# feldroop/genedex

Measured on AMD Instinct MI355X. Metric: queries/sec (count+locate), hg38-scale text, 100M len-50 reads, higher is better.
Workload: dtype u32

## Files before the change

genedex_amd/csrc/search.hip:

```cpp
#include <atomic>
#include <cstdlib>
#include <string>
#include <type_traits>

#include "common.hpp"
#include "kernels.hpp"

namespace gdx {

namespace {

constexpr int kBlock = 256;

struct QueryWindow {
    const uint64_t *words;
    uint64_t cur;
    uint64_t next;
    uint64_t cur_word;
    uint64_t first_word;

    __device__ __forceinline__ void init(const uint8_t *qbuf, uint64_t begin, uint64_t pos)
    {
        words = reinterpret_cast<const uint64_t *>(qbuf);
        first_word = begin >> 3;
// ... 1744 lines not shown
                        a0 = w.l0;
                        a1 = w.l1;
                        a2 = w.l2;
                    }
                    const uint32_t n_lv = rem >> 3 < static_cast<uint32_t>(kLevels) ? rem >> 3 : static_cast<uint32_t>(kLevels);
                    const uint32_t qa = a0, qb = a1 & 0xffffu, qc = __builtin_amdgcn_alignbit(a2, a1, 16);
                    const uint32_t qok = vl & ((1u << n_lv) - 1u);
                    const uint32_t row = lo + sub < hi ? lo + sub : hi - 1u;
                    const u32x4 *tab = static_cast<const u32x4 *>(ix.jump);
                    const u32x4 *pa = kJump == 8 ? tab + (row >> 1) : tab + static_cast<uint64_t>(row) * (kJump / 16);
                    u32x4 e0, e1;
                    load_round2<0>(pa, pa + 1, kHalf2 ? __ballot(true) : 0ull, e0, e1);
                    uint32_t valid, da, db = 0, dc = 0;
                    if (kJump == 8) {
                        const uint32_t ew = (row & 1u) ? e0.w : e0.y;
                        da = (ew ^ qa) & 0xffffu;
                        valid = ew >> 16;
                    } else {
                        da = e0.z ^ qa;
                        db = (e0.w ^ qb) & 0xffffu;
                        valid = e0.w >> 16;
                        if (kHalf2) dc = e1.w ^ qc;
                    }
                    uint32_t good = (da & 0xffffu) == 0u ? 1u : 0u;
                    if (kLevels >= 2) good |= (da >> 16) == 0u ? 2u : 0u;
                    if (kHalf2) {
                        good |= db == 0u ? 4u : 0u;
                        good |= (dc & 0xffffu) == 0u ? 8u : 0u;
                    }
                    good &= valid & qok;
                    const uint32_t lvl = static_cast<uint32_t>(__builtin_ctz(~good | (1u << kLevels)));
                    const uint32_t best = group_max<kGroup>(lvl);
                    if (best == 0u) {
                        jump_ok = false;
                        continue;
                    }
                    const bool mine = lvl == best;
                    uint32_t target = kJump == 8 ? ((row & 1u) ? e0.z : e0.x) : e0.x;
                    if (kLevels >= 2) target = best == 2u ? e0.y : target;
                    if (kHalf2) {
                        target = best == 3u ? e1.x : target;
                        target = best == 4u ? e1.y : target;
                    }
                    lo = group_min<kGroup>(mine ? target : 0xffffffffu);
                    hi = group_max<kGroup>(mine ? target : 0u) + 1u;
                    rem -= best * kJumpSymbols;
                    shift += best;
                    continue;
                }
                const uint32_t e = sel4(shift >> 1, w.l0, w.l1, w.l2, w.l3);
                const uint32_t f = sel4((shift >> 1) + 1u, w.l0, w.l1, w.l2, w.l3);
                const uint32_t lv2 = (shift & 1u) ? ((e & 0xffff0000u) | (f & 0xffffu)) : __builtin_amdgcn_alignbit(e, e, 16);
                const uint32_t x = lv2 << (2u * part);
                const bool two = rem >= 2u;
                {
                    const uint32_t t_last = part + (two ? 1u : 0u);
                    const uint32_t need = (part < w.s0 ? 1u : 2u) | (t_last < w.s0 ? 1u : 2u);
                    if ((v8 & need) != need) {
                        bail = true;
                        break;
                    }
                }
                const uint32_t c1 = (x >> 30) + 1u, c2 = two ? ((x >> 28) & 3u) + 1u : 0u;
                const uint32_t line_lo = lo >> kPairLineShift, line_hi = hi >> kPairLineShift;
                const bool second = line_hi != line_lo;
                const u32x4 *pa = ix.pair_lines + (static_cast<uint64_t>(line_lo) << 3) + sub;
                const u32x4 *pb = ix.pair_lines + (static_cast<uint64_t>(line_hi) << 3) + sub;
                u32x4 a[2], b[2];
                load_round4<0>(pa, pa + kGroup, pb, pb + kGroup, __ballot(true), __ballot(second), a[0], a[1], b[0], b[1]);
                if (!second) {
                    b[0] = a[0];
                    b[1] = a[1];
                }
                bool stepped = false;
                if (two) {
                    const uint32_t pair = (c2 - 1u) * 4u + (c1 - 1u);
                    const uint32_t bits_x = (c1 & 1u) | ((c1 & 2u) << 7) | ((c1 & 4u) << 14) | ((c2 & 1u) << 24);
                    const uint32_t bits_y = ((c2 >> 1) & 1u) | ((c2 & 4u) << 6);
                    const uint32_t nx = ~(bits_x * 0xffu);
                    const uint32_t ny = ~(bits_y * 0xffu) & 0xffffu;
                    uint32_t plo = 0, phi = 0;
#pragma unroll
                    for (int k = 0; k < 2; k++) {
                        plo += PairTable::pair_partial(a[k], sub + k * kGroup, pair, nx, ny, lo);
                        phi += PairTable::pair_partial(b[k], sub + k * kGroup, pair, nx, ny, hi);
                    }
                    const uint32_t nlo = quad_sum(plo), nhi = quad_sum(phi);
                    if (nlo != nhi) {
                        lo = nlo;
                        hi = nhi;
                        rem -= 2u;
                        part += 2u;
                        stepped = true;
                    }
                }
                if (!stepped) {
                    const uint32_t bits_x = (c1 & 1u) | ((c1 & 2u) << 7) | ((c1 & 4u) << 14);
                    const uint32_t nx = ~(bits_x * 0xffu) & 0xffffffu;
                    uint32_t plo = 0, phi = 0;
#pragma unroll
                    for (int k = 0; k < 2; k++) {
                        plo += PairTable::single_partial(a[k], sub + k * kGroup, c1, nx, lo);
                        phi += PairTable::single_partial(b[k], sub + k * kGroup, c1, nx, hi);
                    }
                    lo = quad_sum(plo);
                    hi = quad_sum(phi);
                    rem -= 1u;
                    part += 1u;
                }
                shift += part >> 3;
                part &= 7u;
            }
            if (writer) {
                if (bail) {
                    s_left[atomicAdd(&s_nleft, 1u)] = q;
                } else {
                    const bool unchanged = kCursor && len == 0u;
                    if (out_start && !unchanged) out_start[q] = lo;
                    if (out_end && !unchanged) out_end[q] = hi;
                    if (out_count) out_count[q] = hi - lo;
                    if (!kCursor && out_status) out_status[q] = 0;
                    if (kCursor && ca.active_out != nullptr && lo != hi && more_left) s_alive[slot] = q;
                }
            }
        }
        }
        __syncthreads();
        const uint32_t n_left = s_nleft;
        if (threadIdx.x == 0 && n_left != 0u) s_left_base = atomicAdd(n_leftover, n_left);
        __syncthreads();
        for (uint32_t i = threadIdx.x; i < n_left; i += kBlock) leftover[s_left_base + i] = s_left[i];
        __syncthreads();
        if (threadIdx.x == 0) s_nleft = 0;
        if (kCursor && ca.active_out != nullptr)
            flush_live_ordered(s_alive, cnt, s_alive_part, &s_alive_base, ca.active_out, ca.n_active_out);
    }
}

struct VerifyView {
    const uint2 *top;
    const u32x4 *text_units;
    const uint32_t *sa_full;
    const void *jump;
    const u32x4 *lines;
    const uint32_t *sb_offsets, *count, *sa_samples, *border_keys, *border_vals;
    const uint8_t *io_to_dense;
    uint32_t top_depth, n, n_texts, sa_inv, sa_rot, sa_limit, max_rows;
    uint32_t perm_code_lo, perm_code_hi, perm_exp_lo, perm_exp_hi, perm_mask;
    const u32x4 *seed;
    uint32_t seed_buckets, seed_k, seed_tag_bits;
    const u32x4 *seed_pairs, *seed_quads;
};

template <int kXlate, bool kSeed>
__global__ __launch_bounds__(kBlock) __attribute__((amdgpu_waves_per_eu(7, 7))) void search_verify_kernel4(
    VerifyView vv, const uint8_t *__restrict__ qbuf, const uint64_t *__restrict__ qbeg, const uint64_t *__restrict__ qend,
    uint64_t nq, uint32_t *__restrict__ out_count, uint8_t *__restrict__ out_status, uint4 *out_rec,
    uint32_t range, uint32_t *__restrict__ leftover, uint32_t *__restrict__ n_leftover,
    const uint32_t *__restrict__ list, const uint32_t *__restrict__ n_list,
    uint32_t ulen,
    const uint4 *state,
    uint32_t wide_to_list,
    uint32_t state_packed)
{
    constexpr int kGroup = 4;
    __shared__ uint8_t s_dense[256];
    __shared__ uint32_t s_count[8];
    __shared__ uint32_t s_left[kMaxRange];
    __shared__ uint32_t s_nleft, s_left_base;
    if (list != nullptr) nq = *n_list;
    if (static_cast<uint64_t>(blockIdx.x) * range >= nq) return;
    if (kXlate == 0)
        for (int i = threadIdx.x; i < 256; i += kBlock) s_dense[i] = vv.io_to_dense[i];
    if (threadIdx.x < 8) s_count[threadIdx.x] = threadIdx.x < 6 ? vv.count[threadIdx.x] : 0u;
    if (threadIdx.x == 0) s_nleft = 0;
    __syncthreads();
    IndexView ix{};
    ix.lines = vv.lines;
    ix.sb_offsets = vv.sb_offsets;
    ix.sa_inv = vv.sa_inv;
    ix.sa_rot = vv.sa_rot;
    ix.sa_limit = vv.sa_limit;
    const bool writer = (threadIdx.x % kGroup) == 0;
    const uint32_t sub = threadIdx.x & (kGroup - 1u);
    const uint32_t depth = vv.top_depth;
    const uint64_t n_ranges = (nq + range - 1) / range;
    for (uint64_t rg = blockIdx.x; rg < n_ranges; rg += gridDim.x) {
        const uint64_t base = rg * range;
        const uint32_t cnt = nq - base < range ? static_cast<uint32_t>(nq - base) : range;
        for (uint32_t slot = threadIdx.x / kGroup; slot < cnt; slot += kBlock / kGroup) {
            const uint32_t q = list != nullptr ? list[base + slot] : static_cast<uint32_t>(base + slot);
            uint4 st = make_uint4(0u, 0u, 0u, 0u);
            if (kSeed && state != nullptr) st = state[q];
            const bool from_state = kSeed && state != nullptr && state_packed != 0u && wide_to_list != 0u && (st.y & kStatePacked) != 0u &&
                                    (st.y & kStateSymbolsMask) <= 32u;
            const uint64_t begin = from_state ? 0ull : query_begin(qbeg, ulen, q);
            const uint64_t len = from_state ? 0ull : query_end(qend, ulen, q) - begin;
            bool bail = from_state ? false
                                   : (kSeed ? !(len >= vv.seed_k && len < (1ull << 21)) : !(len >= 16u && len >= depth && len < (1ull << 21)));
            uint32_t lo = 0, hi = 0, rem = 0;
            const uint64_t *wbase = query_words<kXlate>(qbuf, begin);
            const uint32_t off0 = static_cast<uint32_t>(begin & 7u);
            FastWindow w = {0u, 0u, 0u, 0u, 0u, 8u};
            uint32_t shift = 0, part = 0;
            bool single = false;
            bool single_ok = false;
            uint32_t pos = 0;
            bool resumed = false;
            const uint64_t state_codes = (static_cast<uint64_t>(st.z) << 32) | st.w;
            if (from_state && (st.y & kStatePair) != 0u && (st.y >> kStateRowsShift) > 2u) {
                const u32x4 *qr = vv.seed_quads + 4ull * st.x;
                const u32x4 q0 = qr[0], q1 = qr[1], q2 = qr[2], q3 = qr[3];
                const uint32_t n_v = st.y & kStateSymbolsMask, rows_q = st.y >> kStateRowsShift;
                const uint64_t vm64 = n_v == 32u ? ~0ull : ~0ull << (2u * (32u - n_v));
                const uint32_t p_me = sel4(sub, q0.x, q0.y, q0.z, q0.w);
                const uint64_t t_me = (static_cast<uint64_t>(sel4(sub, q1.y, q1.w, q2.y, q2.w)) << 32) | sel4(sub, q1.x, q1.z, q2.x, q2.z);
                uint32_t alive_q = (sub < rows_q && ((state_codes ^ t_me) & vm64) == 0ull && p_me >= n_v) ? 1u << sub : 0u;
                alive_q |= static_cast<uint32_t>(__builtin_amdgcn_mov_dpp(static_cast<int>(alive_q), 0xB1, 0xF, 0xF, true));
                alive_q |= static_cast<uint32_t>(__builtin_amdgcn_mov_dpp(static_cast<int>(alive_q), 0x4E, 0xF, 0xF, true));
                if (writer) {
                    const uint32_t n_alive = static_cast<uint32_t>(__popc(alive_q));
                    uint4 rec;
                    if (n_alive == 0u) {
                        rec = make_uint4(0u, 0u, 0xffffffffu, 0u);
                    } else if (n_alive <= 2u) {
                        const uint32_t f = static_cast<uint32_t>(__builtin_ctz(alive_q));
                        const uint32_t h1 = sel4(f, q0.x, q0.y, q0.z, q0.w) - n_v;
                        if (n_alive == 1u) {
                            rec = make_uint4(0u, 1u, h1, kRecResolved);
                        } else {
                            const uint32_t g = static_cast<uint32_t>(__builtin_ctz(alive_q & (alive_q - 1u)));
                            const uint32_t h2 = sel4(g, q0.x, q0.y, q0.z, q0.w) - n_v;
                            rec = make_uint4(h2, h2 + 2u, h1, kRecResolved);
                        }
                    } else {
                        rec = make_uint4(q3.x, q3.x + n_alive, alive_q, (n_v & 0x1fffffu) | kRecMasked);
                    }
                    if (out_rec) out_rec[q] = rec;
                    if (out_count) out_count[q] = rec.y - rec.x;
                    if (out_status) out_status[q] = 0;
                }
                continue;
            }
            if (from_state && (st.y & kStatePair) != 0u) {
                const u32x4 *pr = vv.seed_pairs + 2ull * st.x;
                const u32x4 r0 = pr[0], r1 = pr[1];
                const uint32_t n_v = st.y & kStateSymbolsMask;
                const uint64_t vm64 = n_v == 32u ? ~0ull : ~0ull << (2u * (32u - n_v));
                const uint64_t t1 = (static_cast<uint64_t>(r0.w) << 32) | r0.z, t2 = (static_cast<uint64_t>(r1.y) << 32) | r1.x;
                const bool ok1 = ((state_codes ^ t1) & vm64) == 0ull && r0.x >= n_v, ok2 = ((state_codes ^ t2) & vm64) == 0ull && r0.y >= n_v;
                if (writer) {
                    const uint32_t h1 = r0.x - n_v, h2 = r0.y - n_v;
                    uint4 rec;
                    if (ok1 && ok2) rec = make_uint4(h2, h2 + 2u, h1, kRecResolved);
                    else if (ok1 || ok2) rec = make_uint4(0u, 1u, ok1 ? h1 : h2, kRecResolved);
                    else rec = make_uint4(0u, 0u, 0xffffffffu, 0u);
                    if (out_rec) out_rec[q] = rec;
                    if (out_count) out_count[q] = rec.y - rec.x;
                    if (out_status) out_status[q] = 0;
                }
                continue;
            }
            if (from_state) {
                resumed = true;
                lo = st.x;
                hi = lo + (st.y >> kStateRowsShift);
                rem = st.y & kStateSymbolsMask;
            } else if (kSeed && !bail && state != nullptr) {
                const bool plain = state_packed == 0u && st.w == 1u;
                const bool p_rows = state_packed != 0u && (st.y & kStatePacked) != 0u, p_wide = state_packed != 0u && (st.y & kStatePlain) != 0u;
                if (plain || p_rows || p_wide) {
                    resumed = true;
                    rem = static_cast<uint32_t>(len);
                    w = fast_window<kXlate>(vv, s_dense, wbase, off0, rem, sub);
                    lo = st.x;
                    hi = plain ? st.y : (p_rows ? lo + (st.y >> kStateRowsShift) : st.z);
                    rem = plain ? st.z : st.y & kStateSymbolsMask;
                    shift = vv.seed_k >> 3;
                    part = vv.seed_k & 7u;
                }
            }
            if (kSeed && !bail && !resumed) {
                rem = static_cast<uint32_t>(len);
                w = fast_window<kXlate>(vv, s_dense, wbase, off0, rem, sub);
                const uint32_t k = vv.seed_k;
                const uint32_t n_look = rem < k + 32u ? rem : k + 32u;
                const uint32_t n_words = n_look <= w.s0 ? 1u : 1u + ((n_look - w.s0 + 7u) >> 3);
                if ((w.valid8 & ((1u << n_words) - 1u)) != (1u << n_words) - 1u) {
                    bail = true;
                } else {
                    const uint32_t w0 = __builtin_amdgcn_alignbit(w.l0, w.l0, 16), w1 = __builtin_amdgcn_alignbit(w.l1, w.l1, 16);
                    const uint32_t w2 = __builtin_amdgcn_alignbit(w.l2, w.l2, 16), w3 = __builtin_amdgcn_alignbit(w.l3, w.l3, 16);
                    const uint64_t key = ((static_cast<uint64_t>(w0) << 32) | w1) >> (64u - 2u * k);
                    uint32_t tag;
                    uint32_t b = seed_home(key, vv.seed_tag_bits, vv.seed_buckets, tag);
                    uint32_t ex, ey, ez, ew;
                    for (uint32_t d = 0;; d++) {
                        const u32x4 *bp = vv.seed + (static_cast<uint64_t>(b) << 3) + 2u * sub;
                        const u32x4 e0 = bp[0], e1 = bp[1];
                        const uint32_t want = tag | (d << kSeedDispShift);
                        const bool m0 = (e0.x & kSeedMatchMask) == want, m1 = (e1.x & kSeedMatchMask) == want;
                        const u32x4 es = m0 ? e0 : e1;
                        const bool m = m0 || m1;
                        ex = m ? (es.x | kSeedFound) : (e0.x & kSeedOverflow);
                        ey = m ? es.y : 0u;
                        ez = m ? es.z : 0u;
                        ew = m ? es.w : 0u;
                        ex |= static_cast<uint32_t>(__builtin_amdgcn_mov_dpp(static_cast<int>(ex), 0xB1, 0xF, 0xF, true));
                        ey |= static_cast<uint32_t>(__builtin_amdgcn_mov_dpp(static_cast<int>(ey), 0xB1, 0xF, 0xF, true));
                        ez |= static_cast<uint32_t>(__builtin_amdgcn_mov_dpp(static_cast<int>(ez), 0xB1, 0xF, 0xF, true));
                        ew |= static_cast<uint32_t>(__builtin_amdgcn_mov_dpp(static_cast<int>(ew), 0xB1, 0xF, 0xF, true));
                        ex |= static_cast<uint32_t>(__builtin_amdgcn_mov_dpp(static_cast<int>(ex), 0x4E, 0xF, 0xF, true));
                        ey |= static_cast<uint32_t>(__builtin_amdgcn_mov_dpp(static_cast<int>(ey), 0x4E, 0xF, 0xF, true));
                        ez |= static_cast<uint32_t>(__builtin_amdgcn_mov_dpp(static_cast<int>(ez), 0x4E, 0xF, 0xF, true));
                        ew |= static_cast<uint32_t>(__builtin_amdgcn_mov_dpp(static_cast<int>(ew), 0x4E, 0xF, 0xF, true));
                        if ((ex & kSeedFound) != 0u || (ex & kSeedOverflow) == 0u || d >= kSeedMaxDisp) break;
                        b = b + 1u == vv.seed_buckets ? 0u : b + 1u;
                    }
                    rem -= k;
                    shift = k >> 3;
                    part = k & 7u;
                    if ((ex & kSeedFound) == 0u) {
                        lo = hi = 0u;
                    } else if ((ex & kSeedKind) != 0u) {
                        lo = ey;
                        hi = ez;
                    } else {
                        single = true;
                        lo = 0u;
                        hi = 1u;
                        pos = ey;
                        uint32_t qh, ql;
                        const uint32_t sh = 32u - 2u * (k & 15u);
                        if (k == 16u) {
                            qh = w1;
                            ql = w2;
                        } else if (k < 16u) {
                            qh = __builtin_amdgcn_alignbit(w0, w1, sh);
                            ql = __builtin_amdgcn_alignbit(w1, w2, sh);
                        } else {
                            qh = __builtin_amdgcn_alignbit(w1, w2, sh);
                            ql = __builtin_amdgcn_alignbit(w2, w3, sh);
                        }
                        const uint32_t n_v = rem < 32u ? rem : 32u;
                        const uint64_t vm64 = n_v == 32u ? ~0ull : ~(~0ull >> (2u * n_v));
                        const uint64_t qcode = (static_cast<uint64_t>(qh) << 32) | ql;
                        const uint64_t tcode = (static_cast<uint64_t>(ew) << 32) | ez;
                        const uint32_t v_code = (ex >> kSeedPartialShift) & 3u;
                        const uint32_t n_text = (ex & kSeedPartial) == 0u ? 0xffffffffu : (v_code == 0u ? (ez & 63u) : 29u + v_code);
                        single_ok = ((qcode ^ tcode) & vm64) == 0ull && pos >= rem && rem <= n_text;
                    }
                }
            }
            if (!kSeed && !bail) {
                rem = static_cast<uint32_t>(len);
                w = fast_window<kXlate>(vv, s_dense, wbase, off0, rem, sub);
                const uint32_t need = (w.s0 == 8u ? 1u : 3u) | (depth > 8u ? (w.s0 == 8u ? 2u : 6u) : 0u);
                if ((w.valid8 & need) != need) {
                    bail = true;
                } else {
                    const uint2 e = vv.top[__builtin_amdgcn_alignbit(w.l0, w.l0, 16) >> (32u - 2u * depth)];
                    lo = e.x;
                    hi = e.y;
                    rem -= depth;
                    shift = depth >> 3;
                    part = depth & 7u;
                }
            }
            if (wide_to_list != 0u && !bail && rem > 0u && hi - lo > vv.max_rows) bail = true;
            while (!bail && rem > 0u && hi - lo > vv.max_rows) {
                if (shift > 6u) {
                    w = fast_window<kXlate>(vv, s_dense, wbase, off0, rem, sub);
                    shift = 0;
                    part = 0;
                }
                const uint32_t v8 = w.valid8 >> shift;
                if ((v8 & (part < w.s0 ? 1u : 2u)) == 0u) {
                    bail = true;
                    break;
                }
                const uint32_t e = sel4(shift >> 1, w.l0, w.l1, w.l2, w.l3);
                const uint32_t lv = (shift & 1u) ? e >> 16 : e & 0xffffu;
                const uint32_t c = ((lv >> (14u - 2u * part)) & 3u) + 1u;
                uint32_t rlo, rhi;
                QuadLineTable::rank2(ix, c, lo, hi, rlo, rhi);
                lo = s_count[c] + rlo;
                hi = s_count[c] + rhi;
                rem--;
                part++;
                shift += part >> 3;
                part &= 7u;
            }
            const uint32_t rows = hi - lo;
            uint32_t alive = 0;
            uint32_t pair_first = 0, pair_second = 0;
            bool pair = false;
            if (kSeed && single && !bail && (rem <= 32u || !single_ok)) {
                alive = single_ok ? 1u : 0u;
            } else if (!bail && rem > 0u && rows != 0u) {
                const bool real = sub < rows;
                const uint32_t row = real ? lo + sub : lo;
                if (kSeed && single) {
                } else if (vv.sa_full != nullptr) {
                    pos = vv.sa_full[row];
                } else if (vv.jump != nullptr) {
                    pos = static_cast<const uint32_t *>(vv.jump)[static_cast<uint64_t>(row) * 8u + 6u];
                } else {
                    uint32_t r_ = row, steps = 0;
                    for (;;) {
                        uint32_t slot_;
                        if (sampled_slot(ix, r_, slot_)) {
                            pos = vv.sa_samples[slot_] + steps;
                            break;
                        }
                        uint32_t rk;
                        const uint32_t c = LineTable::symbol_and_rank(ix, r_, rk);
                        if (c == 0) {
                            pos = vv.border_vals[lower_bound_u32(vv.border_keys, vv.n_texts, r_)] + steps;
                            break;
                        }
                        r_ = vv.count[c] + rk;
                        steps++;
                    }
                }
                bool ok = real && pos >= rem;
                uint32_t rem_v = rem;
                bool first = part == 0u && shift <= 3u;
                if (kSeed && single) {
                    rem_v = rem - 32u;
                    first = false;
                }
                while (rem_v > 0u) {
                    const uint32_t n_v = rem_v < 32u ? rem_v : 32u;
                    uint64_t qcode;
                    if (from_state) {
                        qcode = state_codes;
                    } else {
                        if (!first) {
                            w = fast_window<kXlate>(vv, s_dense, wbase, off0, rem_v, sub);
                            shift = 0;
                        }
                        first = false;
                        const uint32_t v8 = w.valid8 >> shift;
                        const uint32_t vl = v8 & (w.s0 == 8u ? 0xffu : (v8 >> 1));
                        const uint32_t n_full = n_v >> 3, n_tail = n_v & 7u;
                        bool clean = (vl & ((1u << n_full) - 1u)) == ((1u << n_full) - 1u);
                        if (n_tail != 0u) clean = clean && ((v8 >> n_full) & 1u) != 0u && (n_tail <= w.s0 || ((v8 >> (n_full + 1u)) & 1u) != 0u);
                        if (!clean) {
                            bail = true;
                            break;
                        }
                        uint32_t a0, a1;
                        if (shift == 0u) {
                            a0 = w.l0;
                            a1 = w.l1;
                        } else if (shift == 1u) {
                            a0 = __builtin_amdgcn_alignbit(w.l1, w.l0, 16);
                            a1 = __builtin_amdgcn_alignbit(w.l2, w.l1, 16);
                        } else if (shift == 2u) {
                            a0 = w.l1;
                            a1 = w.l2;
                        } else {
                            a0 = __builtin_amdgcn_alignbit(w.l2, w.l1, 16);
                            a1 = __builtin_amdgcn_alignbit(w.l3, w.l2, 16);
                        }
                        qcode = (static_cast<uint64_t>(__builtin_amdgcn_alignbit(a0, a0, 16)) << 32) |
                                static_cast<uint64_t>(__builtin_amdgcn_alignbit(a1, a1, 16));
                    }
                    const uint64_t s0 = static_cast<uint64_t>(pos) - rem + rem_v + 32u * kTextPadUnits - 32u;
                    const uint32_t b = static_cast<uint32_t>(s0 & 31u);
                    const u32x4 *tu = vv.text_units + (s0 >> 5);
                    const u32x4 u0 = ok ? tu[0] : u32x4{0u, 0u, 0u, 0u};
                    const u32x4 u1 = (ok && b != 0u) ? tu[1] : u32x4{0u, 0u, 0u, 0u};
                    const uint64_t c0 = static_cast<uint64_t>(u0.x) | (static_cast<uint64_t>(u0.y) << 32);
                    const uint64_t c1 = static_cast<uint64_t>(u1.x) | (static_cast<uint64_t>(u1.y) << 32);
                    const uint64_t tcode = b ? (c0 >> (2u * b)) | (c1 << (64u - 2u * b)) : c0;
                    const uint32_t tmask = b ? (u0.z >> b) | (u1.z << (32u - b)) : u0.z;
                    const uint64_t vm64 = n_v == 32u ? ~0ull : ~0ull << (2u * (32u - n_v));
                    const uint32_t vm32 = n_v == 32u ? ~0u : ~0u << (32u - n_v);
                    ok = ok && ((qcode ^ tcode) & vm64) == 0ull && (tmask & vm32) == 0u;
                    rem_v -= n_v;
                }
                alive = (ok && !bail) ? 1u << sub : 0u;
                alive |= static_cast<uint32_t>(__builtin_amdgcn_mov_dpp(static_cast<int>(alive), 0xB1, 0xF, 0xF, true));
                alive |= static_cast<uint32_t>(__builtin_amdgcn_mov_dpp(static_cast<int>(alive), 0x4E, 0xF, 0xF, true));
                const int mine = static_cast<int>(pos - rem);
                const uint32_t o0 = static_cast<uint32_t>(__builtin_amdgcn_mov_dpp(mine, 0x00, 0xF, 0xF, true));
                const uint32_t o1 = static_cast<uint32_t>(__builtin_amdgcn_mov_dpp(mine, 0x55, 0xF, 0xF, true));
                const uint32_t o2 = static_cast<uint32_t>(__builtin_amdgcn_mov_dpp(mine, 0xAA, 0xF, 0xF, true));
                const uint32_t o3 = static_cast<uint32_t>(__builtin_amdgcn_mov_dpp(mine, 0xFF, 0xF, 0xF, true));
                if (__popc(alive) == 2) {
                    const uint32_t f = static_cast<uint32_t>(__builtin_ctz(alive)), g = static_cast<uint32_t>(__builtin_ctz(alive & (alive - 1u)));
                    pair_first = sel4(f, o0, o1, o2, o3);
                    pair_second = sel4(g, o0, o1, o2, o3);
                    pair = true;
                }
            }
            if (writer) {
                if (bail) {
                    s_left[atomicAdd(&s_nleft, 1u)] = q;
                    if (kSeed && state_packed != 0u && resumed && out_rec) out_rec[q] = make_uint4(lo, hi, rem, 1u);
                } else {
                    uint4 rec;
                    if (kSeed && single) {
                        rec = alive ? make_uint4(0u, 1u, pos - rem, kRecResolved) : make_uint4(0u, 0u, 0xffffffffu, 0u);
                    } else if (rem == 0u || rows == 0u) {
                        rec = make_uint4(lo, hi, 0xffffffffu, 0u);
                    } else if (rows == 1u) {
                        rec = alive ? make_uint4(lo, lo + 1u, pos - rem, kRecResolved) : make_uint4(lo, lo, 0xffffffffu, 0u);
                    } else if (pair) {
                        rec = make_uint4(pair_second, pair_second + 2u, pair_first, kRecResolved);
                    } else {
                        rec = make_uint4(lo, lo + static_cast<uint32_t>(__popc(alive)), alive, (rem & 0x1fffffu) | kRecMasked);
                    }
                    if (out_rec) out_rec[q] = rec;
                    if (out_count) out_count[q] = rec.y - rec.x;
                    if (out_status) out_status[q] = 0;
                }
            }
        }
        __syncthreads();
        const uint32_t n_left = s_nleft;
        if (threadIdx.x == 0 && n_left != 0u) s_left_base = atomicAdd(n_leftover, n_left);
        __syncthreads();
        for (uint32_t i = threadIdx.x; i < n_left; i += kBlock) leftover[s_left_base + i] = s_left[i];
        __syncthreads();
        if (threadIdx.x == 0) s_nleft = 0;
    }
}

struct SeedView {
    const u32x4 *seed;
    const u32x4 *text_units;
    const uint32_t *isa;
    const uint8_t *io_to_dense;
    uint32_t buckets, k, tag_bits;
    uint32_t perm_code_lo, perm_code_hi, perm_exp_lo, perm_exp_hi, perm_mask;
    uint32_t n = 0;
};

template <int kXlate, bool kExact, bool kCursor = false>
__global__ __launch_bounds__(kBlock) __attribute__((amdgpu_waves_per_eu(8, 8))) void search_seed_kernel4(
    SeedView sv, const uint8_t *__restrict__ qbuf, const uint64_t *__restrict__ qbeg, const uint64_t *__restrict__ qend,
    uint64_t nq, uint32_t *__restrict__ out_count, uint8_t *__restrict__ out_status, uint4 *__restrict__ out_rec,
    uint32_t *__restrict__ out_start, uint32_t *__restrict__ out_end,
    uint32_t range, uint32_t *__restrict__ leftover, uint32_t *__restrict__ n_leftover,
    uint4 *__restrict__ state,
    uint32_t *__restrict__ out_compact,
    uint32_t *__restrict__ long_list, uint32_t *__restrict__ n_long, uint2 *__restrict__ long_state, uint32_t long_stride,
    uint32_t state_packed,
    uint32_t ulen,
    CursorArgs ca)
{
    static_assert(!kCursor || kExact, "cursor chunks are exact searches");
    constexpr uint32_t kGroup = 4, kGroups = kBlock / kGroup;
    constexpr uint32_t kNoQuery = 0xffffffffu;
    __shared__ uint8_t s_dense[256];
    __shared__ uint16_t s_left[kMaxRange], s_long[kMaxRange];
    __shared__ uint32_t s_nleft, s_left_base, s_nlong, s_long_base;
    __shared__ uint32_t s_alive[kCursor ? kCursorRange : 1];
    __shared__ uint32_t s_alive_part[kCursor ? kBlock : 1];
    __shared__ uint32_t s_alive_base;
    if (kXlate == 0)
        for (int i = threadIdx.x; i < 256; i += kBlock) s_dense[i] = sv.io_to_dense[i];
    if (kCursor)
        for (uint32_t i = threadIdx.x; i < kCursorRange; i += kBlock) s_alive[i] = kDeadCursor;
    if (threadIdx.x == 0) s_nleft = s_nlong = 0;
    __syncthreads();
    const uint32_t *active = kCursor ? ca.active_in : nullptr;
    if (kCursor && ca.n_active_in != nullptr) nq = *ca.n_active_in;
    const bool writer = (threadIdx.x % kGroup) == 0;
    const uint32_t sub = threadIdx.x & (kGroup - 1u);
    const uint32_t slot0 = threadIdx.x / kGroup;
    const uint32_t k = sv.k;
    const uint64_t n_ranges = (nq + range - 1) / range;
    for (uint64_t rg = blockIdx.x; rg < n_ranges; rg += gridDim.x) {
        const uint64_t base = rg * range;
        const uint32_t cnt = nq - base < range ? static_cast<uint32_t>(nq - base) : range;
        const int n_it = static_cast<int>((cnt + kGroups - 1u) / kGroups);
        uint64_t c_beg = 0, c_end = 0;
        bool c_on = false;
        u32x4 b_raw = {0u, 0u, 0u, 0u};
        uint64_t b_beg = 0;
        uint32_t b_len = kNoQuery;
        u32x4 a_e0 = {0u, 0u, 0u, 0u}, a_e1 = {0u, 0u, 0u, 0u};
        uint32_t a_tag = 0, a_bucket = 0, a_qh = 0, a_ql = 0, a_rem = kNoQuery;
        bool a_left = false;
        uint32_t z_row = 0, z_q = 0;
        bool z_on = false;
        uint32_t c_q = 0, b_q = 0, a_q = 0, z_slot = 0;
        bool c_more = false, c_ok = true, b_more = false, a_more = false, z_more = false;
        for (int it = -3; it <= n_it; it++) {
            if (kExact) {
                if (z_on && writer) {
                    out_start[z_q] = z_row;
                    out_end[z_q] = z_row + 1u;
                    if (out_count) out_count[z_q] = 1u;
                    if (!kCursor && out_status) out_status[z_q] = 0;
                    if (kCursor && ca.active_out != nullptr && z_more) s_alive[z_slot] = z_q;
                }
                z_on = false;
            }
            if (it == n_it) break;
            if (it >= 0) {
                const uint32_t slot = slot0 + static_cast<uint32_t>(it) * kGroups;
                const uint32_t q = kCursor ? a_q : static_cast<uint32_t>(base + slot);
                if (a_left) {
                    if (writer) {
                        s_left[atomicAdd(&s_nleft, 1u)] = static_cast<uint16_t>(slot);
                        if (state) state[q] = make_uint4(0u, 0u, 0u, 0u);
                        if (!kExact && out_compact) out_compact[q] = kCompactSee;
                    }
                } else if (a_rem != kNoQuery) {
                    uint32_t ex, ey, ez, ew;
                    u32x4 e0 = a_e0, e1 = a_e1;
                    uint32_t b = a_bucket;
                    for (uint32_t d = 0;; d++) {
                        const uint32_t want = a_tag | (d << kSeedDispShift);
                        const bool m0 = (e0.x & kSeedMatchMask) == want, m1 = (e1.x & kSeedMatchMask) == want;
                        const u32x4 es = m0 ? e0 : e1;
                        const bool m = m0 || m1;
                        ex = m ? (es.x | kSeedFound) : (e0.x & kSeedOverflow);
                        ey = m ? es.y : 0u;
                        ez = m ? es.z : 0u;
                        ew = m ? es.w : 0u;
                        ex |= static_cast<uint32_t>(__builtin_amdgcn_mov_dpp(static_cast<int>(ex), 0xB1, 0xF, 0xF, true));
                        ey |= static_cast<uint32_t>(__builtin_amdgcn_mov_dpp(static_cast<int>(ey), 0xB1, 0xF, 0xF, true));
                        ez |= static_cast<uint32_t>(__builtin_amdgcn_mov_dpp(static_cast<int>(ez), 0xB1, 0xF, 0xF, true));
                        ew |= static_cast<uint32_t>(__builtin_amdgcn_mov_dpp(static_cast<int>(ew), 0xB1, 0xF, 0xF, true));
                        ex |= static_cast<uint32_t>(__builtin_amdgcn_mov_dpp(static_cast<int>(ex), 0x4E, 0xF, 0xF, true));
                        ey |= static_cast<uint32_t>(__builtin_amdgcn_mov_dpp(static_cast<int>(ey), 0x4E, 0xF, 0xF, true));
                        ez |= static_cast<uint32_t>(__builtin_amdgcn_mov_dpp(static_cast<int>(ez), 0x4E, 0xF, 0xF, true));
                        ew |= static_cast<uint32_t>(__builtin_amdgcn_mov_dpp(static_cast<int>(ew), 0x4E, 0xF, 0xF, true));
                        if ((ex & kSeedFound) != 0u || (ex & kSeedOverflow) == 0u || d >= kSeedMaxDisp) break;
                        b = b + 1u == sv.buckets ? 0u : b + 1u;
                        const u32x4 *bp = sv.seed + (static_cast<uint64_t>(b) << 3) + 2u * sub;
                        e0 = bp[0];
                        e1 = bp[1];
                    }
                    if ((ex & kSeedFound) != 0u && (ex & kSeedKind) != 0u) {
                        if (kExact && a_rem == 0u) {
                            if (writer) {
                                out_start[q] = ey;
                                out_end[q] = ez;
                                if (out_count) out_count[q] = ez - ey;
                                if (!kCursor && out_status) out_status[q] = 0;
                                if (kCursor && ca.active_out != nullptr && a_more && ey != ez) s_alive[slot] = q;
                            }
                        } else if (writer) {
                            s_left[atomicAdd(&s_nleft, 1u)] = static_cast<uint16_t>(slot);
                            if (!kExact && state) {
                                if (state_packed == 0u) state[q] = make_uint4(ey, ez, a_rem, 1u);
                                else if (state_packed == 2u && (ex & (kSeedPairInfo | kSeedQuadInfo)) != 0u && a_rem - 1u < 32u)
                                    state[q] = make_uint4(ew, ((ez - ey) << kStateRowsShift) | kStatePacked | kStatePair | a_rem, a_qh, a_ql);
                                else if (ez - ey < 256u) state[q] = make_uint4(ey, ((ez - ey) << kStateRowsShift) | kStatePacked | a_rem, a_qh, a_ql);
                                else state[q] = make_uint4(ey, kStatePlain | a_rem, ez, 0u);
                            }
                            if (!kExact && out_compact) out_compact[q] = kCompactSee;
                        }
                    } else {
                        bool hit = false, left = false, is_long = false;
                        const uint32_t rem = a_rem, pos = ey;
                        if ((ex & kSeedFound) != 0u) {
                            const uint32_t n_v = rem < 32u ? rem : 32u;
                            const uint64_t vm64 = n_v == 32u ? ~0ull : ~(~0ull >> (2u * n_v));
                            const uint64_t qcode = (static_cast<uint64_t>(a_qh) << 32) | a_ql;
                            const uint64_t tcode = (static_cast<uint64_t>(ew) << 32) | ez;
                            const uint32_t v_code = (ex >> kSeedPartialShift) & 3u;
                            const uint32_t n_text = (ex & kSeedPartial) == 0u ? 0xffffffffu : (v_code == 0u ? (ez & 63u) : 29u + v_code);
                            hit = ((qcode ^ tcode) & vm64) == 0ull && pos >= rem && rem <= n_text;
                            is_long = hit && rem > 32u;
                        }
// ... 1060 lines not shown
{
    SearchCall c;
    c.d_qbuf = d_qbuf;
    c.d_qbeg = d_qoff;
    c.d_qend = d_qoff + 1;
    c.nq = nq;
    c.d_start = d_out_start;
    c.d_end = d_out_end;
    c.d_count = d_out_count;
    c.d_status = d_out_status;
    c.d_hint = d_hint;
    c.d_step_stats = d_step_stats;
    launch_search_call(ix, c, stream, qo);
}

struct ZeroSegments {
    uint32_t *p[ZeroSet::kMax];
    uint32_t end[ZeroSet::kMax];
    int n;
};
__global__ __launch_bounds__(kBlock) void zero_segments_kernel(ZeroSegments z)
{
    const uint32_t total = z.end[z.n - 1];
    for (uint32_t i = blockIdx.x * kBlock + threadIdx.x; i < total; i += gridDim.x * kBlock) {
        int s = 0;
        while (i >= z.end[s]) s++;
        z.p[s][i - (s == 0 ? 0u : z.end[s - 1])] = 0u;
    }
}

void ZeroSet::add(void *ptr, size_t bytes)
{
    if (ptr == nullptr || bytes == 0) return;
    if (n == kMax || (reinterpret_cast<uintptr_t>(ptr) & 3u) != 0 || bytes > 0xfffffff0ull)
        fail(GDX_ERR_INVALID_ARGUMENT, "internal: ZeroSet takes up to %d 4-byte aligned regions", kMax);
    p[n] = static_cast<uint32_t *>(ptr);
    words[n] = static_cast<uint32_t>((bytes + 3) / 4);
    n++;
}

void ZeroSet::flush(hipStream_t stream)
{
    if (n == 0) return;
    ZeroSegments z{};
    uint64_t total = 0;
    for (int i = 0; i < n; i++) {
        z.p[i] = p[i];
        total += words[i];
        if (total > 0xffffffffull) fail(GDX_ERR_INVALID_ARGUMENT, "internal: ZeroSet regions beyond 16 GB");
        z.end[i] = static_cast<uint32_t>(total);
    }
    z.n = n;
    const uint64_t blocks = (total + kBlock * 4 - 1) / (kBlock * 4);
    hipLaunchKernelGGL(zero_segments_kernel, dim3(static_cast<unsigned>(blocks < 1024 ? blocks : 1024)), dim3(kBlock), 0, stream, z);
    n = 0;
}

__global__ __launch_bounds__(kBlock) void fill_uniform_offsets_kernel(uint64_t *__restrict__ off, uint64_t n, uint32_t ulen)
{
    const uint64_t stride = static_cast<uint64_t>(gridDim.x) * kBlock;
    for (uint64_t i = static_cast<uint64_t>(blockIdx.x) * kBlock + threadIdx.x; i < n; i += stride) off[i] = i * ulen;
}

__global__ __launch_bounds__(kBlock) void fill_uniform_offsets_list_kernel(uint64_t *__restrict__ off, const uint32_t *__restrict__ list,
                                                                          const uint32_t *__restrict__ n_list, uint32_t ulen)
{
    const uint64_t n = *n_list;
    for (uint64_t i = static_cast<uint64_t>(blockIdx.x) * kBlock + threadIdx.x; i < n; i += static_cast<uint64_t>(gridDim.x) * kBlock) {
        const uint64_t q = list[i];
        off[q] = q * ulen;
        off[q + 1] = (q + 1) * ulen;
    }
}

__global__ __launch_bounds__(kBlock) void tile_sums_lists_kernel(const uint4 *__restrict__ rec, const uint32_t *__restrict__ compact,
                                                                 uint32_t max_hits, const uint32_t *__restrict__ left,
                                                                 const uint32_t *__restrict__ n_left, const uint32_t *__restrict__ lng,
                                                                 const uint32_t *__restrict__ n_lng,
                                                                 unsigned long long *__restrict__ tile_sums,
                                                                 unsigned long long *__restrict__ rest)
{
    const uint64_t stride = static_cast<uint64_t>(gridDim.x) * kBlock;
    const uint64_t nl = *n_left, ng = *n_lng;
    const uint64_t n = nl + ng, n_round = (n + 63) / 64 * 64;
    unsigned long long open_slots = 0;
    for (uint64_t i = static_cast<uint64_t>(blockIdx.x) * kBlock + threadIdx.x; i < n_round; i += stride) {
        unsigned long long c = 0;
        uint32_t tile = 0xffffffffu;
        if (i < n) {
            const bool is_left = i < nl;
            const uint32_t q = is_left ? left[i] : lng[i - nl];
            const uint32_t c4 = compact[q];
            tile = q / kSumTile;
            if (c4 == kCompactSee) {
                if (is_left) {
                    const uint2 v = *reinterpret_cast<const uint2 *>(rec + q);
                    const uint32_t m = v.y - v.x;
                    c = (max_hits != 0u && m > max_hits) ? 0ull : static_cast<unsigned long long>(m);
                    open_slots += c;
                }
            } else {
                c = c4 == kCompactNone ? 0ull : 1ull;
            }
        }
        const uint32_t tile0 = static_cast<uint32_t>(__builtin_amdgcn_readfirstlane(static_cast<int>(tile)));
        if (__ballot(tile != tile0 && c != 0ull) == 0ull) {
            unsigned long long sum = tile == tile0 ? c : 0ull;
            for (int off = 32; off > 0; off >>= 1) sum += __shfl_xor(sum, off);
            if ((threadIdx.x & 63u) == 0u && sum != 0ull && tile0 != 0xffffffffu) atomicAdd(&tile_sums[tile0], sum);
        } else if (c != 0ull) {
            atomicAdd(&tile_sums[tile], c);
        }
    }
    for (int off = 32; off > 0; off >>= 1) open_slots += __shfl_xor(open_slots, off);
    if ((threadIdx.x & 63u) == 0u && open_slots != 0ull) atomicAdd(rest, open_slots);
}

template <int V, int... Rest, class F>
static void with_int(int v, F &&f)
{
    if constexpr (sizeof...(Rest) != 0) {
        if (v != V) return with_int<Rest...>(v, f);
    }
    f(std::integral_constant<int, V>());
}
template <class F> static void with_bool(bool b, F &&f) { b ? f(std::true_type()) : f(std::false_type()); }
template <class F> static void with_jump_bytes(int jump_bytes, F &&f) { with_int<32, 16, 8>(jump_bytes, f); }
template <class F> static void with_xlate(int xlate, F &&f) { with_int<2, 1, 0>(xlate, f); }

static int env_int(const char *name, int absent) { const char *e = getenv(name); return e ? atoi(e) : absent; }
static long env_long(const char *name, long absent) { const char *e = getenv(name); return e ? atol(e) : absent; }
static bool env_set(const char *name) { return getenv(name) != nullptr; }

struct SearchKnobs {
    long grid = env_long("GDX_SEARCH_GRID", 0);
    unsigned pad = static_cast<unsigned>(env_long("GDX_SEARCH_PAD", 0));
    int lanes = env_int("GDX_SEARCH_LANES", 4) == 8 ? 8 : 4;
    int policy = env_int("GDX_LOAD_POLICY", 0);
    int schedule = [] { const char *e = getenv("GDX_SEARCH_SCHEDULE"); return (e && e[0] == '0') ? 0 : 1; }();
    int defer = env_int("GDX_SEARCH_DEFER", 0);
    int fast = env_int("GDX_SEARCH_FAST", -1);
    int exact = env_int("GDX_SEARCH_EXACT", -1);
    int seed = env_int("GDX_SEARCH_SEED", -1);
    int text = env_int("GDX_SEARCH_TEXT", 1);
    bool no_perm = env_set("GDX_SEARCH_NO_PERM");
    bool fast_stats = env_set("GDX_SEARCH_FAST_STATS");
    int seed_lean = env_int("GDX_SEARCH_SEED_LEAN", 1);
    int seed_chain = env_int("GDX_SEARCH_SEED_CHAIN", 1);
    int seed_packed = env_int("GDX_SEARCH_SEED_PACKED", 1);
    int seed_lane = env_int("GDX_SEED_LANE", 1);
    int seed_cursor = env_int("GDX_SEARCH_SEED_CURSOR", 1);
    unsigned seed_pad = static_cast<unsigned>(env_long("GDX_SEED_PAD", 0));
    uint32_t seed_lane_range = static_cast<uint32_t>(env_long("GDX_SEED_LANE_RANGE", 0));
    unsigned seed_list_blocks = static_cast<unsigned>(env_long("GDX_SEED_LIST_BLOCKS", 1792));
};
static const SearchKnobs &search_knobs() { static const SearchKnobs knobs; return knobs; }

struct SearchSettings {
    int variant;
    int lanes;
    int policy;
    int schedule;
    uint32_t defer_after;
    int fast;
    bool exact;
    bool seed;
    bool perm;
    int xlate;
    bool text_route;

    SearchSettings(const IndexView &ix, const QueryOptions &qo, const SearchKnobs &k, const SearchCall &c)
    {
        variant = qo.search_variant >= 0 ? qo.search_variant : search_variant();
        lanes = (qo.search_lanes == 4 || qo.search_lanes == 8) ? qo.search_lanes : k.lanes;
        policy = (qo.load_policy >= 0 ? qo.load_policy : k.policy) == 1 ? 1 : 0;
        schedule = qo.length_schedule >= 0 ? (qo.length_schedule != 0) : k.schedule;
        defer_after = c.d_step_stats != nullptr ? 0u : static_cast<uint32_t>(qo.search_defer_after >= 0 ? qo.search_defer_after : k.defer);
        const int f = k.fast >= 0 ? k.fast : qo.search_fast;
        fast = f == 0 ? 0 : (f == 2 ? 2 : 1);
        exact = k.exact >= 0 ? k.exact != 0 : qo.search_exact != 0;
        seed = k.seed >= 0 ? k.seed != 0 : qo.search_seed != 0;
        perm = ix.perm_ok && !k.no_perm;
        xlate = c.packed ? 2 : (perm ? 1 : 0);
        text_route = ix.jump == nullptr && ix.sa_full != nullptr && ix.isa != nullptr && ix.text_units != nullptr && k.text != 0;
    }
};

struct ListGrid { unsigned blocks; uint32_t range; };
static unsigned range_blocks(uint64_t nq, uint32_t range, uint64_t cap)
{
    const uint64_t ranges = (nq + range - 1) / range;
    return static_cast<unsigned>(ranges < cap ? ranges : cap);
}
static ListGrid range_grid(uint64_t nq, uint32_t range_cap, long grid_override)
{
    uint64_t per_block = (nq + 1791) / 1792;
    per_block = (per_block + 63) / 64 * 64;
    const uint32_t range = static_cast<uint32_t>(per_block > range_cap ? range_cap : per_block);
    return {grid_override > 0 ? static_cast<unsigned>(grid_override) : range_blocks(nq, range, 1u << 20), range};
}
static ListGrid short_list_grid(uint64_t nq, unsigned cap = 8192) { return {range_blocks(nq, 256, cap), 256}; }
static unsigned group_grid(uint64_t nq, uint64_t groups_per_block, long grid_override)
{
    const uint64_t needed = (nq + groups_per_block - 1) / groups_per_block;
    uint64_t blocks = (nq + groups_per_block * 48 - 1) / (groups_per_block * 48);
    if (blocks < 1792) blocks = 1792;
    if (blocks > 65536) blocks = 65536;
    if (blocks > needed) blocks = needed;
    if (grid_override > 0) blocks = static_cast<uint64_t>(grid_override);
    return static_cast<unsigned>(blocks);
}

static SeedView seed_view(const IndexView &ix, const uint32_t *isa)
{
    return SeedView{ix.seed, ix.text_units, isa, ix.io_to_dense, ix.seed_buckets, ix.seed_k, ix.seed_tag_bits,
                    ix.perm_code_lo, ix.perm_code_hi, ix.perm_exp_lo, ix.perm_exp_hi, ix.perm_mask};
}
static VerifyView verify_view(const IndexView &ix)
{
    const bool entry_sa = ix.jump != nullptr && ix.jump_bytes == 32;
    const uint32_t max_rows = (ix.sa_full != nullptr || entry_sa) ? 4u : 1u;
    return VerifyView{ix.top, ix.text_units, ix.sa_full, entry_sa ? ix.jump : nullptr, ix.lines, ix.sb_offsets, ix.count,
                      ix.sa_samples, ix.border_keys, ix.border_vals, ix.io_to_dense, ix.top_depth, ix.n, ix.n_texts,
                      ix.sa_inv, ix.sa_rot, ix.sa_limit, max_rows, ix.perm_code_lo, ix.perm_code_hi, ix.perm_exp_lo,
                      ix.perm_exp_hi, ix.perm_mask, ix.seed, ix.seed_buckets, ix.seed_k, ix.seed_tag_bits, ix.seed_pairs, ix.seed_quads};
}
static ExactView exact_view(const IndexView &ix, bool with_seed)
{
    return ExactView{ix.top, ix.jump, ix.pair_lines, ix.io_to_dense, ix.top_depth, ix.n, static_cast<uint32_t>(ix.depth),
                     ix.perm_code_lo, ix.perm_code_hi, ix.perm_exp_lo, ix.perm_exp_hi, ix.perm_mask, ix.sa_full, ix.isa,
                     ix.text_units, with_seed ? ix.seed : nullptr, ix.seed_buckets, ix.seed_k, ix.seed_tag_bits};
}
static FastView fast_view(const IndexView &ix)
{
    return FastView{ix.top, ix.jump, ix.io_to_dense, ix.top_depth, ix.sa_inv, ix.sa_rot, ix.sa_limit,
                    ix.perm_code_lo, ix.perm_code_hi, ix.perm_exp_lo, ix.perm_exp_hi, ix.perm_mask};
}

struct SeedLaunch {
    SeedView sv;
    ListGrid grid;
    unsigned lds = 0;
    uint4 *rec = nullptr;
    uint32_t *start = nullptr, *end = nullptr;
    uint32_t *first = nullptr, *lng = nullptr;
    uint4 *state = nullptr;
    uint32_t *compact = nullptr;
    uint2 *long_state = nullptr;
    uint32_t long_stride = 0, state_packed = 0;
};

struct SearchChain {
    ZeroSet zs;
    CursorArgs ca;
    bool leftover_list = false;
    uint32_t *seed_list = nullptr;
    uint32_t seed_state_packed = 0;
    bool compact_by_seed = false;
    uint32_t *fold_left = nullptr, *fold_long = nullptr;
    uint64_t *d_uniform_off = nullptr;
    bool sparse_offsets = false;
    ListGrid all{}, exact{}, general{};
    CursorArgs ca_exact, ca_general;
};

struct SearchLauncher {
    const IndexView &ix;
    SearchCall c;
    hipStream_t stream;
    const SearchKnobs &k;
    const SearchSettings s;
    const uint64_t nq;
    const bool seed_pairs;
    const long lane_blocks_cap;
    uint32_t ulen = 0;
    SearchChain st;

    uint32_t *counted_list(int slot, ZeroSet *zs)
    {
        uint32_t *list = static_cast<uint32_t *>(stream_scratch(stream, slot, (nq + 4) * sizeof(uint32_t)));
        if (zs != nullptr) zs->add(list, sizeof(uint32_t));
        else GDX_HIP(hipMemsetAsync(list, 0, sizeof(uint32_t), stream));
        return list;
    }
    void print_left(const char *path, const uint32_t *n_list, const char *next)
    {
        uint32_t n_left = 0;
        GDX_HIP(hipMemcpyAsync(&n_left, n_list, sizeof(uint32_t), hipMemcpyDeviceToHost, stream));
        GDX_HIP(hipStreamSynchronize(stream));
        fprintf(stderr, "gdx: %s path left %u of %llu queries to the %s kernel\n", path, n_left, static_cast<unsigned long long>(nq), next);
    }
    template <int kXlate, bool kExact>
    void launch_seed_text(const SeedLaunch &a)
    {
        hipLaunchKernelGGL((seed_text_kernel4<kXlate, kExact>), dim3(range_blocks(nq, kBlock / 4, 8192)), dim3(kBlock), 0, stream, a.sv,
                           c.d_qbuf, c.d_qbeg, a.lng + 4, a.lng, a.long_state, a.long_stride, c.d_count, c.d_status, a.rec, a.start,
                           a.end, a.compact, a.state, a.first + 4, a.first, ulen);
    }
    template <int kXlate, bool kExact>
    void launch_seed_and_text(const SeedLaunch &a)
    {
        hipLaunchKernelGGL((search_seed_kernel4<kXlate, kExact>), dim3(a.grid.blocks), dim3(kBlock), a.lds, stream, a.sv, c.d_qbuf,
                           c.d_qbeg, c.d_qend, nq, c.d_count, c.d_status, a.rec, a.start, a.end, a.grid.range, a.first + 4, a.first,
                           a.state, a.compact, a.lng + 4, a.lng, a.long_state, a.long_stride, a.state_packed, ulen, CursorArgs());
        launch_seed_text<kXlate, kExact>(a);
    }
    template <bool kSeed>
// ... 465 lines not shown
```

Measured before the change: 26.00 billion.

## Software-pipeline verify kernel loads across list, state, record, and decision stages

Restructures the per-query loop of the verify kernel into a four-stage software pipeline: list entry, packed state, and the seed pair/quad record are prefetched for later slots while an earlier slot's decision runs. This overlaps dependent global-memory loads. Each lane now loads only its own slice of the quad record rather than all four vectors. It also rebalances the per-block range for list-driven launches, lowers waves-per-EU for the seed variant to 5 and sets the default list block count to match. The cost is more live registers and lower occupancy, which could offset the latency hiding.

```diff
diff --git a/genedex_amd/csrc/search.hip b/genedex_amd/csrc/search.hip
--- a/genedex_amd/csrc/search.hip
+++ b/genedex_amd/csrc/search.hip
@@ -1920,8 +1920,38 @@
     const u32x4 *seed_pairs, *seed_quads;
 };
 
+constexpr uint32_t kVerifyDepth = 4;
+constexpr int kVerifySeedWaves = 5;
+template <bool kSeed>
+__device__ __forceinline__ bool verify_from_state(const uint4 *state, uint32_t state_packed, uint32_t wide_to_list, const uint4 &st)
+{
+    return kSeed && state != nullptr && state_packed != 0u && wide_to_list != 0u && (st.y & kStatePacked) != 0u &&
+           (st.y & kStateSymbolsMask) <= 32u;
+}
+struct VerifyRecord {
+    u32x4 a;
+    uint2 b;
+    uint32_t c;
+};
+__device__ __forceinline__ VerifyRecord verify_record_load(const u32x4 *seed_pairs, const u32x4 *seed_quads, const uint4 &st, uint32_t sub)
+{
+    VerifyRecord r;
+    if ((st.y >> kStateRowsShift) > 2u) {
+        const u32x4 *qr = seed_quads + 4ull * st.x;
+        r.a = qr[0];
+        r.b = reinterpret_cast<const uint2 *>(qr + 1)[sub];
+        r.c = reinterpret_cast<const uint32_t *>(qr + 3)[0];
+    } else {
+        const u32x4 *pr = seed_pairs + 2ull * st.x;
+        r.a = pr[0];
+        r.b = reinterpret_cast<const uint2 *>(pr + 1)[0];
+        r.c = 0u;
+    }
+    return r;
+}
+
 template <int kXlate, bool kSeed>
-__global__ __launch_bounds__(kBlock) __attribute__((amdgpu_waves_per_eu(7, 7))) void search_verify_kernel4(
+__global__ __launch_bounds__(kBlock) __attribute__((amdgpu_waves_per_eu(kSeed ? kVerifySeedWaves : 7, kSeed ? kVerifySeedWaves : 7))) void search_verify_kernel4(
     VerifyView vv, const uint8_t *__restrict__ qbuf, const uint64_t *__restrict__ qbeg, const uint64_t *__restrict__ qend,
     uint64_t nq, uint32_t *__restrict__ out_count, uint8_t *__restrict__ out_status, uint4 *out_rec,
     uint32_t range, uint32_t *__restrict__ leftover, uint32_t *__restrict__ n_leftover,
@@ -1936,7 +1966,14 @@
     __shared__ uint32_t s_count[8];
     __shared__ uint32_t s_left[kMaxRange];
     __shared__ uint32_t s_nleft, s_left_base;
-    if (list != nullptr) nq = *n_list;
+    if (list != nullptr) {
+        nq = *n_list;
+        const uint64_t per = (nq + gridDim.x - 1) / gridDim.x;
+        if (per > range) {
+            const uint64_t rounds = (per + kMaxRange - 1) / kMaxRange;
+            range = static_cast<uint32_t>(((per + rounds - 1) / rounds + 63u) & ~63ull);
+        }
+    }
     if (static_cast<uint64_t>(blockIdx.x) * range >= nq) return;
     if (kXlate == 0)
         for (int i = threadIdx.x; i < 256; i += kBlock) s_dense[i] = vv.io_to_dense[i];
@@ -1956,12 +1993,8 @@
     for (uint64_t rg = blockIdx.x; rg < n_ranges; rg += gridDim.x) {
         const uint64_t base = rg * range;
         const uint32_t cnt = nq - base < range ? static_cast<uint32_t>(nq - base) : range;
-        for (uint32_t slot = threadIdx.x / kGroup; slot < cnt; slot += kBlock / kGroup) {
-            const uint32_t q = list != nullptr ? list[base + slot] : static_cast<uint32_t>(base + slot);
-            uint4 st = make_uint4(0u, 0u, 0u, 0u);
-            if (kSeed && state != nullptr) st = state[q];
-            const bool from_state = kSeed && state != nullptr && state_packed != 0u && wide_to_list != 0u && (st.y & kStatePacked) != 0u &&
-                                    (st.y & kStateSymbolsMask) <= 32u;
+        auto decide = [&](const uint32_t q, const uint4 st, const u32x4 ra, const uint2 rb, const uint32_t rc) {
+            const bool from_state = verify_from_state<kSeed>(state, state_packed, wide_to_list, st);
             const uint64_t begin = from_state ? 0ull : query_begin(qbeg, ulen, q);
             const uint64_t len = from_state ? 0ull : query_end(qend, ulen, q) - begin;
             bool bail = from_state ? false
@@ -1977,12 +2010,11 @@
             bool resumed = false;
             const uint64_t state_codes = (static_cast<uint64_t>(st.z) << 32) | st.w;
             if (from_state && (st.y & kStatePair) != 0u && (st.y >> kStateRowsShift) > 2u) {
-                const u32x4 *qr = vv.seed_quads + 4ull * st.x;
-                const u32x4 q0 = qr[0], q1 = qr[1], q2 = qr[2], q3 = qr[3];
+                const u32x4 q0 = ra;
                 const uint32_t n_v = st.y & kStateSymbolsMask, rows_q = st.y >> kStateRowsShift;
                 const uint64_t vm64 = n_v == 32u ? ~0ull : ~0ull << (2u * (32u - n_v));
                 const uint32_t p_me = sel4(sub, q0.x, q0.y, q0.z, q0.w);
-                const uint64_t t_me = (static_cast<uint64_t>(sel4(sub, q1.y, q1.w, q2.y, q2.w)) << 32) | sel4(sub, q1.x, q1.z, q2.x, q2.z);
+                const uint64_t t_me = (static_cast<uint64_t>(rb.y) << 32) | rb.x;
                 uint32_t alive_q = (sub < rows_q && ((state_codes ^ t_me) & vm64) == 0ull && p_me >= n_v) ? 1u << sub : 0u;
                 alive_q |= static_cast<uint32_t>(__builtin_amdgcn_mov_dpp(static_cast<int>(alive_q), 0xB1, 0xF, 0xF, true));
                 alive_q |= static_cast<uint32_t>(__builtin_amdgcn_mov_dpp(static_cast<int>(alive_q), 0x4E, 0xF, 0xF, true));
@@ -2002,20 +2034,19 @@
                             rec = make_uint4(h2, h2 + 2u, h1, kRecResolved);
                         }
                     } else {
-                        rec = make_uint4(q3.x, q3.x + n_alive, alive_q, (n_v & 0x1fffffu) | kRecMasked);
+                        rec = make_uint4(rc, rc + n_alive, alive_q, (n_v & 0x1fffffu) | kRecMasked);
                     }
                     if (out_rec) out_rec[q] = rec;
                     if (out_count) out_count[q] = rec.y - rec.x;
                     if (out_status) out_status[q] = 0;
                 }
-                continue;
+                return;
             }
             if (from_state && (st.y & kStatePair) != 0u) {
-                const u32x4 *pr = vv.seed_pairs + 2ull * st.x;
-                const u32x4 r0 = pr[0], r1 = pr[1];
+                const u32x4 r0 = ra;
                 const uint32_t n_v = st.y & kStateSymbolsMask;
                 const uint64_t vm64 = n_v == 32u ? ~0ull : ~0ull << (2u * (32u - n_v));
-                const uint64_t t1 = (static_cast<uint64_t>(r0.w) << 32) | r0.z, t2 = (static_cast<uint64_t>(r1.y) << 32) | r1.x;
+                const uint64_t t1 = (static_cast<uint64_t>(r0.w) << 32) | r0.z, t2 = (static_cast<uint64_t>(rb.y) << 32) | rb.x;
                 const bool ok1 = ((state_codes ^ t1) & vm64) == 0ull && r0.x >= n_v, ok2 = ((state_codes ^ t2) & vm64) == 0ull && r0.y >= n_v;
                 if (writer) {
                     const uint32_t h1 = r0.x - n_v, h2 = r0.y - n_v;
@@ -2027,7 +2058,7 @@
                     if (out_count) out_count[q] = rec.y - rec.x;
                     if (out_status) out_status[q] = 0;
                 }
-                continue;
+                return;
             }
             if (from_state) {
                 resumed = true;
@@ -2286,6 +2317,29 @@
                     if (out_status) out_status[q] = 0;
                 }
             }
+        };
+        constexpr uint32_t kGroups = kBlock / kGroup;
+        uint32_t q1 = 0, q2 = 0, q3 = 0;
+        uint4 st2 = make_uint4(0u, 0u, 0u, 0u), st3 = st2;
+        VerifyRecord r3 = {};
+        for (uint32_t slot = threadIdx.x / kGroup; slot < cnt + (kVerifyDepth - 1u) * kGroups; slot += kGroups) {
+            const bool v0 = slot < cnt, v1 = slot >= kGroups && slot - kGroups < cnt;
+            const bool v2 = slot >= 2u * kGroups && slot - 2u * kGroups < cnt, v3 = slot >= 3u * kGroups && slot - 3u * kGroups < cnt;
+            uint32_t n1 = 0;
+            if (v0) n1 = list != nullptr ? list[base + slot] : static_cast<uint32_t>(base + slot);
+            uint4 n2 = make_uint4(0u, 0u, 0u, 0u);
+            if (kSeed && state != nullptr && v1) n2 = state[q1];
+            VerifyRecord n3 = {};
+            if (v2 && verify_from_state<kSeed>(state, state_packed, wide_to_list, st2) && (st2.y & kStatePair) != 0u)
+                n3 = verify_record_load(vv.seed_pairs, vv.seed_quads, st2, sub);
+            if (v3) decide(q3, st3, r3.a, r3.b, r3.c);
+            static_assert(kVerifyDepth == 4u, "the stages below are written out: entry, state, record, decision");
+            q3 = q2;
+            st3 = st2;
+            r3 = n3;
+            q2 = q1;
+            st2 = n2;
+            q1 = n1;
         }
         __syncthreads();
         const uint32_t n_left = s_nleft;
@@ -3652,7 +3706,7 @@
     int seed_cursor = env_int("GDX_SEARCH_SEED_CURSOR", 1);
     unsigned seed_pad = static_cast<unsigned>(env_long("GDX_SEED_PAD", 0));
     uint32_t seed_lane_range = static_cast<uint32_t>(env_long("GDX_SEED_LANE_RANGE", 0));
-    unsigned seed_list_blocks = static_cast<unsigned>(env_long("GDX_SEED_LIST_BLOCKS", 1792));
+    unsigned seed_list_blocks = static_cast<unsigned>(env_long("GDX_SEED_LIST_BLOCKS", 256 * kVerifySeedWaves));
 };
 static const SearchKnobs &search_knobs() { static const SearchKnobs knobs; return knobs; }
 
```

Result: no change. 26.26 billion, median of 4 (+1.0%).
